# CatchMan1/AI-education-generative-recommendation

Hardware: AMD Instinct MI355X
Metric: RQ-VAE items encoded/s + SASRec seqs scored/s @1/8 GPU; HR@10/NDCG@10 parity (higher is better)
Workload: dtype f32; 1 GPU; rq_c2: RQ-VAE get_indices, 3x256 codebooks, in 768 -> [256,128] -> e 32, data-derived codebooks, BERT-statistics item embeddings; global_batch=100000, parallelism=item-sharded x1, no collective

## Files before the change

ai-education-generative-recommendation_amd/csrc/abi.cpp:

```cpp
#include <atomic>
#include <cstring>
#include <string>

#include "gr_common.h"

namespace gr {
static thread_local std::string g_last_error;
void set_error(const std::string& msg) { g_last_error = msg; }
void clear_error() { g_last_error.clear(); }

int cu_count() {
  static int cus = 0;
  if (!cus) {
    int dev = 0;
    if (hipGetDevice(&dev) != hipSuccess) dev = 0;
    if (hipDeviceGetAttribute(&cus, hipDeviceAttributeMultiprocessorCount, dev) != hipSuccess || cus < 1)
      cus = 256;
  }
  return cus;
}

struct Opt {
  const char* name;
  std::atomic<int64_t>* v;
  int64_t lo, hi;
};
static std::atomic<int64_t> g_rq_fused{1};
static std::atomic<int64_t> g_sas_fused{2};
static std::atomic<int64_t> g_sas_rowtile{1};
static std::atomic<int64_t> g_lin_wres{1};
static std::atomic<int64_t> g_emb_proj{1};
static std::atomic<int64_t> g_topk_half{2};
static std::atomic<int64_t> g_attn_k16{1};
static std::atomic<int64_t> g_rq_filter{1};
static std::atomic<int64_t> g_rq_tail_merge{1};

static std::atomic<int64_t> g_kmeans_small{1};
static std::atomic<int64_t> g_bert_tile{0};

static const Opt kOpts[] = {
    {"rq_fused", &g_rq_fused, 0, 1},   {"sas_fused", &g_sas_fused, 0, 3}, {"sas_rowtile", &g_sas_rowtile, 0, 1},
    {"lin_wres", &g_lin_wres, 0, 1},   {"emb_proj", &g_emb_proj, 0, 1},   {"topk_half", &g_topk_half, 0, 2},
    {"attn_k16", &g_attn_k16, 0, 1},   {"rq_filter", &g_rq_filter, 0, 1}, {"kmeans_small", &g_kmeans_small, 0, 1},
    {"rq_tail_merge", &g_rq_tail_merge, 0, 1}, {"bert_tile", &g_bert_tile, 0, 3},
};

static const Opt* find_opt(const char* name) {
  for (const Opt& o : kOpts)
    if (!strcmp(name, o.name)) return &o;
  return nullptr;
}

int64_t option(const char* name) {
  const Opt* o = find_opt(name);
  return o ? o->v->load() : -1;
}
}

extern "C" int gr_set_option(const char* name, int64_t value) {
  gr::clear_error();
  if (!name) return gr::fail(GR_ERR_ARG, "gr_set_option: null name");
  const gr::Opt* o = gr::find_opt(name);
  if (!o || value < o->lo || value > o->hi)
    return gr::fail(GR_ERR_ARG, std::string("gr_set_option: unknown option or value: ") + name);
  o->v->store(value);
  return GR_OK;
}

extern "C" int64_t gr_get_option(const char* name) { return name ? gr::option(name) : -1; }

extern "C" const char* gr_version(void) { return "gr_amd 0.1.0 gfx950"; }
extern "C" const char* gr_last_error(void) { return gr::g_last_error.c_str(); }
```

ai-education-generative-recommendation_amd/csrc/rq.hip:

```cpp
#include <atomic>

#include "gr_common.h"
#include "rq_fused.h"
#include "rq_quant.h"

#ifndef GR_QDIAG
#define GR_QDIAG 0
#endif

#ifndef GR_QRES
#define GR_QRES 1
#endif

namespace gr {

struct RQLevels {
  const float* cb[GR_MAX_LEVELS];
  int K[GR_MAX_LEVELS];
};

constexpr int RQ_SPLIT_MAX = 3;
constexpr size_t RQ_PART_BYTES = 2 * RQ_SPLIT_MAX * 4 * 32 * 3 * sizeof(float);

template <int EP>
// ... 118 lines not shown
    }
    __syncthreads();
  }
  int loff = 0;
  for (int l = 0; l < (GR_QDIAG == 5 ? 0 : L); ++l) {
    const int K = lv.K[l];
    const float* cb = lv.cb[l];
    float* cbi = resident ? cbs + loff * EP : cbs;
    float* cni = resident ? cns + loff : cns;
    const int kst = resident ? K : kch;
    loff += (K + 31) & ~31;
    float rn[RQ_MAXT], best[RQ_MAXT], second[RQ_MAXT];
    int bi[RQ_MAXT];
#pragma unroll
    for (int i = 0; i < RQ_MAXT; ++i) {
      rn[i] = GR_QDIAG == 4 ? 0.f : rn_exact<EP>(res[i], e, h);
      best[i] = __builtin_inff();
      second[i] = __builtin_inff();
      bi[i] = 0x7fffffff;
    }
    const int c_last = ((K - 1) / kst) * kst;
    for (int c0 = 0; c0 < K; c0 += kst) {
      const int cnt = min(kst, K - c0);
      if (!resident) {
        __syncthreads();
        stage_codes<EP, NT, FULL>(cb, e, c0, cnt, cbs, cns, tid);
      }
      const int ct_n = (cnt + 31) >> 5;
      const int q_lo = simd * ct_n / 4, q_hi = (simd + 1) * ct_n / 4;
#pragma unroll 1
      for (int ct = 0; ct < ct_n; ++ct) {
        const bool in_q = ct >= q_lo && ct < q_hi;
        const int code = min(ct * 32 + r, cnt - 1);
        f32x4 a[HQ];
#pragma unroll
        for (int j = 0; j < HQ; ++j)
          a[j] = *reinterpret_cast<const f32x4*>(cbi + cb_off<EP>(code, HQ * h + j));
        float cnv[16];
#pragma unroll
        for (int g4 = 0; g4 < 4; ++g4) {
          const f32x4 q = *reinterpret_cast<const f32x4*>(cni + ct * 32 + 8 * g4 + 4 * h);
#pragma unroll
          for (int i = 0; i < 4; ++i) cnv[4 * g4 + i] = q[i];
        }
#pragma unroll
        for (int i = 0; i < RQ_MAXT; ++i) {
          if (i < my && (!is_split(i) || in_q)) {
            f32x16 acc;
#pragma unroll
            for (int v = 0; v < 16; ++v) acc[v] = 0.f;
#pragma unroll
            for (int j = 0; j < HQ; ++j)
#pragma unroll
              for (int s = 0; s < 4; ++s) {
                if (GR_QDIAG == 2) acc[4 * j + s] += a[j][s] * res[i][j][s];
                else acc = mfma32(a[j][s], res[i][j][s], acc);
              }
#pragma unroll
            for (int v = 0; v < 16; ++v) {
              const int cd = c0 + ct * 32 + (v & 3) + 8 * (v >> 2) + 4 * h;
              const float dd = fmaf(-2.f, acc[v], rn[i] + cnv[v]);
              if (GR_QDIAG == 1) {
                best[i] = fminf(best[i], acc[v]);
                continue;
              }
              const bool lt = dd < best[i];
              if (SECOND) second[i] = lt ? best[i] : fminf(second[i], dd);
              bi[i] = lt ? cd : bi[i];
              best[i] = lt ? dd : best[i];
            }
          }
        }
      }
    }
#pragma unroll
    for (int i = 0; i < RQ_MAXT; ++i) {
      if (i < my) {
        const float ob = __shfl_xor(best[i], 32), os = __shfl_xor(second[i], 32);
        const int oi = __shfl_xor(bi[i], 32);
        merge_min<SECOND>(best[i], second[i], bi[i], ob, os, oi);
      }
    }
    if (split_plan) {
      float* pl = part + (l & 1) * (RQ_SPLIT_MAX * 4 * 32 * 3);
#pragma unroll
      for (int i = 0; i < RQ_MAXT; ++i)
        if (i < my && is_split(i) && h == 0) {
          float* ep = pl + (((wk + i * WS - base) * 4 + simd) * 32 + r) * 3;
          ep[0] = best[i];
          ep[1] = second[i];
          ep[2] = __int_as_float(bi[i]);
        }
      __syncthreads();
#pragma unroll
      for (int i = 0; i < RQ_MAXT; ++i)
        if (i < my && is_split(i)) {
          const float* ep = pl + ((wk + i * WS - base) * 4 * 32 + r) * 3;
          float bb = ep[0], ss = ep[1];
          int ii = __float_as_int(ep[2]);
#pragma unroll
          for (int q = 1; q < 4; ++q)
            merge_min<SECOND>(bb, ss, ii, ep[q * 96], ep[q * 96 + 1], __float_as_int(ep[q * 96 + 2]));
          best[i] = bb;
          second[i] = ss;
          bi[i] = ii;
        }
    }
#pragma unroll
    for (int i = 0; i < RQ_MAXT; ++i) {
      if (i < my) {
        int b = bi[i];
        if (b >= K) b = 0;
        const int64_t item = (int64_t)tile_of(i) * 32 + r;
        if (h == 0 && item < n && (!is_split(i) || simd == 0)) {
          idx_out[item * L + l] = (int64_t)b;
          if (best_out) best_out[item * L + l] = best[i];
          if (gap_out) gap_out[item * L + l] = second[i] - best[i];
        }
        f32x4 cw[HQ];
        if (b >= c_last) {
#pragma unroll
          for (int j = 0; j < HQ; ++j)
            cw[j] = *reinterpret_cast<const f32x4*>(cbi + cb_off<EP>(b - c_last, HQ * h + j));
        } else {
#pragma unroll
          for (int j = 0; j < HQ; ++j)
#pragma unroll
            for (int s = 0; s < 4; ++s) {
              const int f = 8 * j + 2 * s + h;
              cw[j][s] = f < e ? cb[(int64_t)b * e + f] : 0.f;
            }
        }
#pragma unroll
        for (int j = 0; j < HQ; ++j)
#pragma unroll
          for (int s = 0; s < 4; ++s) {
            const float xq = res[i][j][s] + (cw[j][s] - res[i][j][s]);
            res[i][j][s] = res[i][j][s] - xq;
          }
      }
    }
  }
}

#ifndef GR_FDIAG
#define GR_FDIAG 0
#endif
#ifndef GR_FSB
#define GR_FSB 1
#endif
#ifndef GR_FLIVE
#define GR_FLIVE 1
#endif

typedef __bf16 bf16x8 __attribute__((ext_vector_type(8)));

constexpr int RQF_KMAX = 1024;
constexpr int RQF_F32_KMAX = 512;

__device__ __forceinline__ void split_bf16(float x, __bf16& hi, __bf16& lo) {
#pragma clang fp contract(off)
  hi = (__bf16)x;
  lo = (__bf16)(x - (float)hi);
}

__device__ __forceinline__ f32x16 filter_tile(const bf16x8 (&ah)[2], const bf16x8 (&al)[2], const bf16x8 (&bh)[2],
                                              const bf16x8 (&bl)[2], f32x16 acc) {
#pragma unroll
  for (int t = 0; t < 2; ++t) acc = __builtin_amdgcn_mfma_f32_32x32x16_bf16(ah[t], bh[t], acc, 0, 0, 0);
#pragma unroll
  for (int t = 0; t < 2; ++t) acc = __builtin_amdgcn_mfma_f32_32x32x16_bf16(ah[t], bl[t], acc, 0, 0, 0);
#pragma unroll
  for (int t = 0; t < 2; ++t) acc = __builtin_amdgcn_mfma_f32_32x32x16_bf16(al[t], bh[t], acc, 0, 0, 0);
  return acc;
}

__host__ __device__ inline size_t filter_lds_floats(int kch, int f32_lds) {
  return ((size_t)kch * 32 * (f32_lds ? 2 : 1) + (size_t)kch + 16 + 255) & ~(size_t)255;
}
#ifndef GR_FDMA
#define GR_FDMA 1
#endif
__device__ __forceinline__ void filter_stage_dma(const float* __restrict__ img, float* buf, int img_floats, int tid) {
  const int w = __builtin_amdgcn_readfirstlane(tid >> 6), lane = tid & 63;
  for (int c = w; c < img_floats / 256; c += RQ_W)
    __builtin_amdgcn_global_load_lds(
        reinterpret_cast<const __attribute__((address_space(1))) void*>(reinterpret_cast<uintptr_t>(img + c * 256 + lane * 4)),
        (__attribute__((address_space(3))) void*)(buf + c * 256), 16, 0, 0);
}
template <bool LIVE>
__device__ __forceinline__ void filter_stage(const float* __restrict__ cb, int K, int kch, int f32_lds, float* sm,
                                             const float* __restrict__ img, int img_floats, int tid) {
#pragma clang fp contract(off)
  constexpr int EP = 32, W = RQ_W, NT = W * 64;
  if (img) {
    for (int f = tid; f < img_floats / 4; f += NT)
      *reinterpret_cast<f32x4*>(sm + 4 * f) = *reinterpret_cast<const f32x4*>(img + 4 * f);
    return;
  }
  float* bimg = sm;
  float* cns = bimg + kch * EP;
  float* wmax = cns + kch;
  float* fimg = wmax + 16;
  const int lane = tid & 63, w = tid >> 6, ct_n = (K + 31) >> 5;
  for (int f = tid; f < 2 * K; f += NT) {
    const int c = f >> 1, t = f & 1;
    float x[16];
#pragma unroll
    for (int q = 0; q < 4; ++q) {
      const f32x4 v = *reinterpret_cast<const f32x4*>(cb + (int64_t)c * EP + 16 * t + 4 * q);
#pragma unroll
      for (int i = 0; i < 4; ++i) x[4 * q + i] = v[i];
    }
#pragma unroll
    for (int hh = 0; hh < 2; ++hh) {
      bf16x8 vh, vl;
#pragma unroll
      for (int i = 0; i < 8; ++i) {
        __bf16 a, b;
        split_bf16(x[(i < 4 ? 2 * i : 8 + 2 * (i - 4)) + hh], a, b);
        vh[i] = a;
        vl[i] = b;
      }
      *reinterpret_cast<bf16x8*>(bimg + cb_off<EP>(c, 2 * hh + t)) = vh;
      *reinterpret_cast<bf16x8*>(bimg + cb_off<EP>(c, 4 + 2 * hh + t)) = vl;
    }
  }
  if (f32_lds) stage_rows<EP, NT, true>(cb, EP, 0, K, fimg, tid);
  float cmax = 0.f;
  for (int c = tid; c < (LIVE ? 256 : ct_n * 32); c += NT) {
    float s = __builtin_inff();
    if (c < K) {
      const float* row = cb + (int64_t)c * EP;
      s = aten_rowsq([&](int f) { return row[f]; }, EP);
      cmax = fmaxf(cmax, s);
    }
    cns[c] = s;
  }
  cmax = xmax<32>(xmax<16>(xmax<8>(xmax<4>(xmax<2>(xmax<1>(cmax))))));
  if (lane == 0) wmax[w] = cmax;
}

template <bool LIVE, bool TAIL, bool DBUF>
__global__ __launch_bounds__(RQ_W * 64) void rq_filter_kernel(
    const float* __restrict__ z, int64_t n, int L, RQLevels lv, int kch, int f32_lds,
    int64_t* __restrict__ idx_out, int tiles, uint32_t* __restrict__ cand_out, RqPending tail,
    const float* __restrict__ img, int img_floats) {
#pragma clang fp contract(off)
  constexpr int EP = 32, HQ = 4, W = RQ_W, MAXT = GR_FMAXT;
  if (LIVE) f32_lds = 1;
  extern __shared__ __attribute__((aligned(16))) float sm[];
  const int tid = threadIdx.x, lane = tid & 63, w = tid >> 6, r = lane & 31, h = lane >> 5;
  const int left = TAIL ? tail.left : 0;
  const bool owner = TAIL && (int)blockIdx.x < left;
  int t_begin, t_end;
  rq_filter_range(tiles, (int)gridDim.x, left, (int)blockIdx.x, t_begin, t_end);
  const int cm = t_end - t_begin, lt = TAIL ? tail.t0 + (int)blockIdx.x : 0;
  const int my = (cm + (owner ? 1 : 0) - w + W - 1) / W;
  auto tile_at = [&](int i) -> int { return (TAIL && w + i * W >= cm) ? lt : t_begin + w + i * W; };

  if constexpr (TAIL) {
    if (owner) {
      using FC = FusedCfg<256, 128>;
      float *h1s = sm, *h2s = h1s + FT * FC::P1, *w3s = h2s + FT * FC::P2;
      rq_leftover_tile<256, 128, true>(tail.h1g + (int64_t)blockIdx.x * FT * 256, n, lt, tail.W2, tail.b2, tail.W3,
                                       tail.b3, tail.z, h1s, h2s, w3s, h1s);
      __syncthreads();
    }
  }

  f32x4 res[MAXT][HQ];
#pragma unroll
  for (int i = 0; i < MAXT; ++i) {
    const int64_t item = (int64_t)tile_at(i) * 32 + r;
    const bool ok = i < my && item < n;
    const int64_t ic = ok ? item : 0;
    if (TAIL && owner && i < my && w + i * W == cm) {
#pragma unroll
      for (int j = 0; j < HQ; ++j) {
        const f32x4 lo = *reinterpret_cast<const f32x4*>(sm + r * ZLP + 8 * j);
        const f32x4 hi = *reinterpret_cast<const f32x4*>(sm + r * ZLP + 8 * j + 4);
        const f32x4 v = h ? f32x4{lo[1], lo[3], hi[1], hi[3]} : f32x4{lo[0], lo[2], hi[0], hi[2]};
        res[i][j] = ok ? v : f32x4{0.f, 0.f, 0.f, 0.f};
      }
      continue;
    }
#pragma unroll
    for (int j = 0; j < HQ; ++j) {
      const f32x4 lo = *reinterpret_cast<const f32x4*>(z + ic * EP + 8 * j);
      const f32x4 hi = *reinterpret_cast<const f32x4*>(z + ic * EP + 8 * j + 4);
      const f32x4 v = h ? f32x4{lo[1], lo[3], hi[1], hi[3]} : f32x4{lo[0], lo[2], hi[0], hi[2]};
      res[i][j] = ok ? v : f32x4{0.f, 0.f, 0.f, 0.f};
    }
  }

  for (int l = 0; l < L; ++l) {
    const int K = lv.K[l];
    const float* __restrict__ cb = lv.cb[l];
    const int ct_n = (K + 31) >> 5;
    if (DBUF) asm volatile("s_waitcnt vmcnt(0)" ::: "memory");
    __syncthreads();
    float* lb = sm;
    if constexpr (DBUF) {
      lb = sm + (l & 1) * img_floats;
      if (l == 0) {
        filter_stage_dma(img, lb, img_floats, tid);
        asm volatile("s_waitcnt vmcnt(0)" ::: "memory");
        __syncthreads();
      }
      if (l + 1 < L) filter_stage_dma(img + (size_t)(l + 1) * img_floats, sm + ((l + 1) & 1) * img_floats, img_floats, tid);
    } else {
      filter_stage<LIVE>(cb, K, kch, f32_lds, sm, img ? img + (size_t)l * img_floats : nullptr, img_floats, tid);
    }
    float* bimg = lb;
    float* cns = bimg + kch * EP;
    float* wmax = cns + kch;
    float* fimg = wmax + 16;
    float cmax = 0.f;
    if (!DBUF) __syncthreads();
#pragma unroll
    for (int i = 0; i < W; ++i) cmax = fmaxf(cmax, wmax[i]);

    float rn[MAXT], m[MAXT];
#pragma unroll
    for (int i = 0; i < MAXT; ++i) {
      if (!LIVE) rn[i] = rn_exact<EP>(res[i], EP, h);
      m[i] = __builtin_inff();
    }
    auto split_res = [&](int i, bf16x8 (&bh)[2], bf16x8 (&bl)[2]) {
#pragma unroll
      for (int t = 0; t < 2; ++t)
#pragma unroll
        for (int q = 0; q < 8; ++q) {
          __bf16 a, b;
          split_bf16(-2.f * res[i][2 * t + (q >> 2)][q & 3], a, b);
          bh[t][q] = a;
          bl[t][q] = b;
        }
    };
    auto load_codes = [&](int ct, bf16x8 (&ah)[2], bf16x8 (&al)[2], f32x16& cnv) {
      const int code = min(ct * 32 + r, K - 1);
#pragma unroll
      for (int t = 0; t < 2; ++t) {
        ah[t] = *reinterpret_cast<const bf16x8*>(bimg + cb_off<EP>(code, 2 * h + t));
        al[t] = *reinterpret_cast<const bf16x8*>(bimg + cb_off<EP>(code, 4 + 2 * h + t));
      }
#pragma unroll
      for (int g4 = 0; g4 < 4; ++g4) {
        const f32x4 q = *reinterpret_cast<const f32x4*>(cns + ct * 32 + 8 * g4 + 4 * h);
#pragma unroll
        for (int i = 0; i < 4; ++i) cnv[4 * g4 + i] = q[i];
      }
    };
    float thr[MAXT], best[MAXT];
    int bi[MAXT];
    bool allm[MAXT];
    uint32_t ncand[MAXT];
#pragma unroll
    for (int i = 0; i < MAXT; ++i) {
      best[i] = __builtin_inff();
      bi[i] = 0x7fffffff;
      ncand[i] = 0;
    }
    auto set_thr = [&](int i) {
      m[i] = fminf(m[i], __shfl_xor(m[i], 32));
      thr[i] = m[i] + 2.f * rq_filter_bound(rn[i], cmax);
      allm[i] = !(fabsf(thr[i]) < __builtin_inff());
      if (GR_FDIAG == 2) bi[i] = __float_as_int(thr[i]) & 0xff;
    };
    auto min16 = [](float t, const f32x16& a) {
#pragma unroll
      for (int v = 0; v < 16; v += 2) t = fminf(fminf(t, a[v]), a[v + 1]);
      return t;
    };
    auto mark16 = [](uint32_t k, const f32x16& a, float th) {
      const f32x16 d = th - a;
#pragma unroll
      for (int v = 0; v < 16; ++v) k = __builtin_amdgcn_alignbit(k, __float_as_uint(d[v]), 31);
      return k;
    };
    auto walk = [&](int i, int g0, const uint32_t (&nm)[4]) {
      if (GR_FDIAG == 1) {
        bi[i] = min(bi[i], (int)((nm[0] ^ nm[1] ^ nm[2] ^ nm[3]) >> 1));
        return;
      }
      uint32_t cm[4];
#pragma unroll
      for (int q = 0; q < 4; ++q) cm[q] = allm[i] ? 0xffffffffu : ~nm[q];
      if (__builtin_amdgcn_ballot_w64((cm[0] | cm[1] | cm[2] | cm[3]) != 0) == 0) return;
      float ev[16], od[16];
#pragma unroll
      for (int j = 0; j < HQ; ++j)
#pragma unroll
        for (int s = 0; s < 4; ++s) {
          const float own = res[i][j][s], oth = __shfl_xor(own, 32);
          ev[4 * j + s] = h ? oth : own;
          od[4 * j + s] = h ? own : oth;
        }
      while (__builtin_amdgcn_ballot_w64((cm[0] | cm[1] | cm[2] | cm[3]) != 0) != 0) {
        const int q = cm[0] ? 0 : cm[1] ? 1 : cm[2] ? 2 : 3;
        const uint32_t wd = cm[0] ? cm[0] : cm[1] ? cm[1] : cm[2] ? cm[2] : cm[3];
        const bool act = wd != 0;
        const int p = 31 - __clz((int)(wd | 1u));
        const uint32_t keep = ~(1u << p);
#pragma unroll
        for (int qq = 0; qq < 4; ++qq) cm[qq] = qq == q ? cm[qq] & keep : cm[qq];
        const int v = 15 - (p & 15);
        const int cd = (g0 + 2 * q + (p < 16 ? 1 : 0)) * 32 + (v & 3) + 8 * (v >> 2) + 4 * h;
        if (act && cd < K) {
          float cr[EP];
          if (f32_lds) {
#pragma unroll
            for (int sl = 0; sl < 2 * HQ; ++sl) {
              const f32x4 t = *reinterpret_cast<const f32x4*>(fimg + cb_off<EP>(cd, sl));
#pragma unroll
              for (int s = 0; s < 4; ++s) cr[8 * (sl % HQ) + 2 * s + sl / HQ] = t[s];
            }
          } else {
#pragma unroll
            for (int sl = 0; sl < EP / 4; ++sl) {
              const f32x4 t = *reinterpret_cast<const f32x4*>(cb + (int64_t)cd * EP + 4 * sl);
#pragma unroll
              for (int s = 0; s < 4; ++s) cr[4 * sl + s] = t[s];
            }
          }
          float chain = 0.f;
#pragma unroll
          for (int k = 0; k < EP; ++k) chain = fmaf(cr[k], (k & 1) ? od[k >> 1] : ev[k >> 1], chain);
          const float dd = fmaf(-2.f, chain, rn[i] + cns[cd]);
          const bool lt = dd < best[i];
          bi[i] = lt ? cd : bi[i];
          best[i] = lt ? dd : best[i];
          ++ncand[i];
        }
      }
    };
    auto finish = [&](int i) {
      float sec = 0.f;
      merge_min<false>(best[i], sec, bi[i], __shfl_xor(best[i], 32), 0.f, __shfl_xor(bi[i], 32));
      int b = bi[i];
      if (b >= K || b < 0) b = 0;
      const int64_t item = (int64_t)tile_at(i) * 32 + r;
      if (h == 0 && item < n) idx_out[item * L + l] = (int64_t)b;
      if (GR_FDIAG == 3) {
        const uint32_t tot = ncand[i] + __shfl_xor(ncand[i], 32);
        if (h == 0 && item < n && cand_out) cand_out[item * L + l] = tot;
      }
      f32x4 cw[HQ];
      if (f32_lds) {
#pragma unroll
        for (int j = 0; j < HQ; ++j) cw[j] = *reinterpret_cast<const f32x4*>(fimg + cb_off<EP>(b, HQ * h + j));
      } else {
#pragma unroll
        for (int j = 0; j < HQ; ++j) {
          const f32x4 lo = *reinterpret_cast<const f32x4*>(cb + (int64_t)b * EP + 8 * j);
          const f32x4 hi = *reinterpret_cast<const f32x4*>(cb + (int64_t)b * EP + 8 * j + 4);
          cw[j] = h ? f32x4{lo[1], lo[3], hi[1], hi[3]} : f32x4{lo[0], lo[2], hi[0], hi[2]};
        }
      }
#pragma unroll
      for (int j = 0; j < HQ; ++j)
#pragma unroll
        for (int s = 0; s < 4; ++s) {
          const float xq = res[i][j][s] + (cw[j][s] - res[i][j][s]);
          res[i][j][s] = res[i][j][s] - xq;
        }
    };
    if constexpr (LIVE) {
#pragma unroll
      for (int i = 0; i < MAXT; ++i) {
        if (i < my && GR_FDIAG == 4) {
          rn[i] = 0.f;
          finish(i);
        } else if (i < my) {
          f32x16 acc[8];
          float t = __builtin_inff();
          bf16x8 bh[2], bl[2];
          split_res(i, bh, bl);
          rn[i] = rn_exact<EP>(res[i], EP, h);
#pragma unroll
          for (int u = 0; u < 8; ++u)
          {
            bf16x8 ah[2], al[2];
            f32x16 cnv;
            load_codes(u, ah, al, cnv);
            acc[u] = filter_tile(ah, al, bh, bl, cnv);
#if GR_FSB
            t = min16(t, acc[u]);
            __builtin_amdgcn_sched_barrier(0);
#endif
          }
#if !GR_FSB
#pragma unroll
          for (int u = 0; u < 8; ++u) t = min16(t, acc[u]);
#endif
          m[i] = t;
          set_thr(i);
          if (GR_FDIAG == 2) {
            finish(i);
            continue;
          }
          uint32_t nm[4];
#pragma unroll
          for (int u = 0; u < 8; ++u) {
            nm[u >> 1] = mark16((u & 1) ? nm[u >> 1] : 0u, acc[u], thr[i]);
            __builtin_amdgcn_sched_barrier(0);
          }
          walk(i, 0, nm);
          finish(i);
        }
      }
    } else {
      bf16x8 bh[MAXT][2], bl[MAXT][2];
#pragma unroll
      for (int i = 0; i < MAXT; ++i) split_res(i, bh[i], bl[i]);
#pragma unroll 1
      for (int ct = 0; ct < (GR_FDIAG == 4 ? 0 : ct_n); ++ct) {
        bf16x8 ah[2], al[2];
        f32x16 cnv;
        load_codes(ct, ah, al, cnv);
#pragma unroll
        for (int i = 0; i < MAXT; ++i)
          if (i < my) m[i] = min16(m[i], filter_tile(ah, al, bh[i], bl[i], cnv));
      }
#pragma unroll
      for (int i = 0; i < MAXT; ++i) set_thr(i);
      for (int g0 = 0; g0 < (GR_FDIAG == 2 || GR_FDIAG == 4 ? 0 : ct_n); g0 += 8) {
        uint32_t nmk[MAXT][4];
#pragma unroll
        for (int u = 0; u < 8; ++u) {
          if (g0 + u < ct_n) {
            bf16x8 ah[2], al[2];
            f32x16 cnv;
            load_codes(g0 + u, ah, al, cnv);
#pragma unroll
            for (int i = 0; i < MAXT; ++i)
              if (i < my)
                nmk[i][u >> 1] = mark16((u & 1) ? nmk[i][u >> 1] : 0u, filter_tile(ah, al, bh[i], bl[i], cnv), thr[i]);
          } else {
#pragma unroll
            for (int i = 0; i < MAXT; ++i) nmk[i][u >> 1] = (((u & 1) ? nmk[i][u >> 1] : 0u) << 16) | 0xffffu;
          }
        }
#pragma unroll
        for (int i = 0; i < MAXT; ++i)
          if (i < my) walk(i, g0, nmk[i]);
      }
#pragma unroll
      for (int i = 0; i < MAXT; ++i)
        if (i < my) finish(i);
    }
  }
}

template <bool LIVE>
__global__ __launch_bounds__(RQ_W * 64) void rq_cb_pack_kernel(RQLevels lv, int kch, int f32_lds,
                                                              float* __restrict__ out, int img_floats) {
  constexpr int W = RQ_W, NT = W * 64;
  extern __shared__ __attribute__((aligned(16))) float sm[];
  const int tid = threadIdx.x, l = blockIdx.x;
  for (int f = tid; f < img_floats; f += NT) sm[f] = 0.f;
  __syncthreads();
  filter_stage<LIVE>(lv.cb[l], lv.K[l], kch, f32_lds, sm, nullptr, 0, tid);
  __syncthreads();
  float* wmax = sm + kch * 32 + kch;
  float cmax = 0.f;
#pragma unroll
  for (int i = 0; i < W; ++i) cmax = fmaxf(cmax, wmax[i]);
  __syncthreads();
  if (tid < 16) wmax[tid] = tid < W ? cmax : 0.f;
  __syncthreads();
  for (int f = tid; f < img_floats; f += NT) out[(size_t)l * img_floats + f] = sm[f];
}

__global__ __launch_bounds__(256) void rq_code_norms_kernel(const float* __restrict__ cb, int K,
                                                            int e, float* __restrict__ cn) {
  const int c = blockIdx.x * 256 + threadIdx.x;
  if (c >= K) return;
  const float* row = cb + (int64_t)c * e;
  cn[c] = aten_rowsq([&](int f) { return row[f]; }, e);
}

static int launch_norms(const float* cb, int K, int e, float* cn, hipStream_t st) {
  hipLaunchKernelGGL(rq_code_norms_kernel, dim3((K + 255) / 256), dim3(256), 0, st, cb, K, e, cn);
  return check_launch("gr_rq_codebook_norms_f32");
}

template <int EP>
static int launch_quantize_e(const float* z, int64_t n, int e, int L, const RQLevels& lv, int64_t* idx,
                             float* best, float* gap, hipStream_t st) {
  int kmax = 0;
  for (int l = 0; l < L; ++l) kmax = lv.K[l] > kmax ? lv.K[l] : kmax;
  const int kch_max = 1024 * 32 / EP;
  int kch = ((kmax < kch_max ? kmax : kch_max) + 31) & ~31;
  const int64_t tiles = (n + 31) / 32;
  int ktot = 0;
  for (int l = 0; l < L; ++l) ktot += (lv.K[l] + 31) & ~31;
  const bool res = GR_QRES && tiles <= (int64_t)cu_count() &&
                   (size_t)ktot * EP * 4 + (size_t)ktot * 4 + RQ_PART_BYTES <= 160 * 1024;
  if (res) kch = ktot;
  const size_t lds = (size_t)kch * EP * 4 + (size_t)kch * 4 + RQ_PART_BYTES;
  int64_t grid = (int64_t)cu_count();
  const int64_t min_grid = (tiles + RQ_W * RQMaxT<EP>::value - 1) / (RQ_W * RQMaxT<EP>::value);
  if (grid < min_grid) grid = min_grid;
  if (grid > tiles) grid = tiles;
  if (grid > 0x7fffffffLL || tiles > 0x7fffffffLL) return fail(GR_ERR_UNSUPPORTED, "rq quantize: n too large");
  const bool full = e == EP;
  auto k = (best || gap) ? (full ? rq_quantize_kernel<EP, true, true> : rq_quantize_kernel<EP, true, false>)
                         : (full ? rq_quantize_kernel<EP, false, true> : rq_quantize_kernel<EP, false, false>);
  if (lds > 64 * 1024 &&
      hipFuncSetAttribute(reinterpret_cast<const void*>(k), hipFuncAttributeMaxDynamicSharedMemorySize,
                          (int)lds) != hipSuccess)
    return fail(GR_ERR_HIP, "rq quantize: cannot raise the LDS limit");
  hipLaunchKernelGGL(k, dim3((unsigned)grid), dim3(RQ_W * 64), lds, st, z, n, e, L, lv, kch, idx,
                     best, gap, (int)tiles, 1, res ? 1 : 0);
  return check_launch("gr_rq_quantize_f32");
}

static std::atomic<int64_t> g_filter_launches{0};
static std::atomic<uint32_t*> g_filter_counts{nullptr};

static bool filter_ok(int e, int L, const RQLevels& lv, const float* best, const float* gap) {
  if (e != 32 || best || gap || option("rq_filter") != 1) return false;
  for (int l = 0; l < L; ++l)
    if (lv.K[l] > RQF_KMAX) return false;
  return true;
}

static int64_t filter_grid(int64_t tiles, int64_t grid_in, int left) {
  const int cap = RQ_W * GR_FMAXT;
  int64_t grid = grid_in;
  const int64_t min_grid = (tiles + cap - 1) / cap;
  if (grid < min_grid) grid = min_grid;
  if (grid < left || left > tiles || tiles > 0x7fffffffLL) return 0;
  while (grid <= 0x7fffffffLL && rq_filter_max_count((int)tiles, (int)grid, left) > cap) ++grid;
  return grid > 0x7fffffffLL ? 0 : grid;
}

struct FilterShape {
  bool live;
  int kch, f32_lds;
  size_t floats;
};
static FilterShape filter_shape(int L, const RQLevels& lv) {
  int kmax = 0;
  for (int l = 0; l < L; ++l) kmax = lv.K[l] > kmax ? lv.K[l] : kmax;
  FilterShape s;
  s.live = GR_FLIVE && kmax <= 256;
  s.kch = s.live ? 256 : (kmax + 31) & ~31;
  s.f32_lds = s.kch <= RQF_F32_KMAX;
  s.floats = filter_lds_floats(s.kch, s.f32_lds);
  return s;
}

static int launch_filter(const float* z, int64_t n, int L, const RQLevels& lv, int64_t* idx, hipStream_t st,
                         const RqPending* tail = nullptr, const float* img = nullptr) {
  const FilterShape fs = filter_shape(L, lv);
  const bool live = fs.live;
  const int kch = fs.kch, f32_lds = fs.f32_lds;
  size_t lds = fs.floats * sizeof(float);
  const bool merged = tail && tail->h1g;
  const bool dbuf = GR_FDMA && live && img && L > 1 && 2 * lds <= 160 * 1024;
  if (dbuf) lds *= 2;
  if (merged && lds < FusedCfg<256, 128>::TAIL_LDS * sizeof(float)) lds = FusedCfg<256, 128>::TAIL_LDS * sizeof(float);
  const int64_t tiles = (n + 31) / 32;
  int64_t grid = (int64_t)cu_count();
  if (grid > tiles) grid = tiles;
  grid = filter_grid(tiles, grid, merged ? tail->left : 0);
  if (grid == 0)
    return fail(GR_ERR_UNSUPPORTED, merged ? "rq encode: n too large (the pending leftover tiles were not finished)"
                                           : "rq quantize: n too large");
  auto k = merged ? (live ? rq_filter_kernel<true, true, false> : rq_filter_kernel<false, true, false>)
                  : (live ? rq_filter_kernel<true, false, false> : rq_filter_kernel<false, false, false>);
#if GR_FDMA
  if (dbuf) k = merged ? rq_filter_kernel<true, true, true> : rq_filter_kernel<true, false, true>;
#endif
  if (lds > 64 * 1024 &&
      hipFuncSetAttribute(reinterpret_cast<const void*>(k),
                          hipFuncAttributeMaxDynamicSharedMemorySize, (int)lds) != hipSuccess)
    return fail(GR_ERR_HIP, merged ? "rq encode: cannot raise the LDS limit (the pending leftover tiles were not finished)"
                                   : "rq quantize: cannot raise the LDS limit");
  hipLaunchKernelGGL(k, dim3((unsigned)grid), dim3(RQ_W * 64), lds, st, z, n, L, lv, kch, f32_lds,
                     idx, (int)tiles, g_filter_counts.load(), merged ? *tail : RqPending{}, img, (int)fs.floats);
  g_filter_launches.fetch_add(1);
  return check_launch("gr_rq_quantize_f32");
}

static int launch_cb_pack(int L, const RQLevels& lv, float* out, hipStream_t st) {
  const FilterShape fs = filter_shape(L, lv);
  auto k = fs.live ? rq_cb_pack_kernel<true> : rq_cb_pack_kernel<false>;
  const size_t lds = fs.floats * sizeof(float);
  if (lds > 64 * 1024 &&
      hipFuncSetAttribute(reinterpret_cast<const void*>(k), hipFuncAttributeMaxDynamicSharedMemorySize, (int)lds) != hipSuccess)
    return fail(GR_ERR_HIP, "rq codebook pack: cannot raise the LDS limit");
  hipLaunchKernelGGL(k, dim3((unsigned)L), dim3(RQ_W * 64), lds, st, lv, fs.kch, fs.f32_lds, out, (int)fs.floats);
  return check_launch("gr_rq_codebook_pack_f32");
}

static int launch_quantize(const float* z, int64_t n, int e, int L, const RQLevels& lv,
                           int64_t* idx, float* best, float* gap, hipStream_t st, const float* img = nullptr) {
  if (n == 0) return GR_OK;
  if (filter_ok(e, L, lv, best, gap)) return launch_filter(z, n, L, lv, idx, st, nullptr, img);
  if (e <= 16) return launch_quantize_e<16>(z, n, e, L, lv, idx, best, gap, st);
  if (e <= 32) return launch_quantize_e<32>(z, n, e, L, lv, idx, best, gap, st);
  if (e <= 64) return launch_quantize_e<64>(z, n, e, L, lv, idx, best, gap, st);
  return fail(GR_ERR_UNSUPPORTED, "gr_rq_quantize_f32: e_dim must be <= 64");
}

static int check_levels(int32_t e, int32_t L, const int32_t* K, const float* const* cbs) {
  if (e < 1 || e > 4096) return fail(GR_ERR_UNSUPPORTED, "rq: 1 <= e_dim <= 4096");
  if (L < 1 || L > GR_MAX_LEVELS) return fail(GR_ERR_UNSUPPORTED, "rq: 1 <= L <= 8 levels");
  if (!K || !cbs) return fail(GR_ERR_ARG, "rq: null K / codebooks");
  for (int l = 0; l < L; ++l) {
    if (K[l] < 1) return fail(GR_ERR_ARG, "rq: codebook size must be >= 1");
    if (!cbs[l] || ((e == 16 || e == 32 || e == 64) && !aligned16(cbs[l]))) return fail(GR_ERR_ARG, "rq: codebooks must be 16-byte aligned");
  }
  return GR_OK;
}

static bool quant_chain(int64_t M, int e, int L, const int32_t* K) {
  if (e > 64) return false;
  for (int l = 0; l < L; ++l) {
    const MklPlan p = mkl_plan(M, e, K[l]);
    if (p.kind != MKL_CHAIN || p.kb < e) return false;
  }
  return true;
}

static bool mlp_chain(int64_t M, int32_t n_linear, const int32_t* dims) {
  for (int i = 0; i < n_linear; ++i) {
    const MklPlan p = mkl_plan(M, dims[i], dims[i + 1]);
    if (p.kind != MKL_CHAIN || p.kb % 2 != 0 || dims[i] % 4 != 0) return false;
  }
  return true;
}

}

extern "C" int32_t gr_mkl_plan(int64_t M, int32_t K, int32_t N, int32_t* kind, int32_t* kb) {
  const gr::MklPlan p = gr::mkl_plan(M, K, N);
  if (kind) *kind = p.kind;
  if (kb) *kb = p.kb;
  return gr::mkl_plan_pinned(M, K, N) ? 1 : 0;
}

extern "C" float gr_rq_filter_bound_f32(float rn, float cmax2) { return gr::rq_filter_bound(rn, cmax2); }

extern "C" int64_t gr_rq_filter_launches(void) { return gr::g_filter_launches.load(); }

extern "C" int gr_rq_filter_plan(int64_t tiles, int32_t grid_in, int32_t left, int32_t* begins_out,
                                 int32_t* counts_out, int32_t* grid_out) {
  using namespace gr;
  clear_error();
  if (tiles < 1 || grid_in < 1 || left < 0 || !grid_out) return fail(GR_ERR_ARG, "gr_rq_filter_plan: bad arguments");
  const int64_t grid = filter_grid(tiles, grid_in, left);
  if (grid == 0) return fail(GR_ERR_UNSUPPORTED, "gr_rq_filter_plan: left > grid or tiles, or too many tiles");
  *grid_out = (int32_t)grid;
  for (int b = 0; b < (int)grid && (begins_out || counts_out); ++b) {
    int mb, me;
    rq_filter_range((int)tiles, (int)grid, left, b, mb, me);
    if (begins_out) begins_out[b] = mb;
    if (counts_out) counts_out[b] = me - mb + (b < left ? 1 : 0);
  }
  return GR_OK;
}

extern "C" void gr_rq_filter_diag_counts(uint32_t* counts) { gr::g_filter_counts.store(counts); }

extern "C" int gr_rq_codebook_norms_f32(const float* codebook, int32_t K, int32_t e, float* cn_out,
                                        void* stream) {
  gr::clear_error();
  if (!codebook || !cn_out || K < 1 || e < 1) return gr::fail(GR_ERR_ARG, "gr_rq_codebook_norms_f32: bad args");
  return gr::launch_norms(codebook, K, e, cn_out, reinterpret_cast<hipStream_t>(stream));
}

extern "C" int gr_rq_quantize_f32(const float* z, int64_t n, int32_t e, int32_t L, const int32_t* K,
                                  const float* const* codebooks, const float* const* code_norms,
                                  int64_t* idx_out, float* best_out, float* gap_out,
                                  void* stream) {
  using namespace gr;
  clear_error();
  (void)code_norms;
  int rc = check_levels(e, L, K, codebooks);
  if (rc) return rc;
  if (n < 0) return fail(GR_ERR_ARG, "gr_rq_quantize_f32: n < 0");
  if (n == 0) return GR_OK;
  if (!z || !idx_out || ((e == 16 || e == 32 || e == 64) && !aligned16(z))) return fail(GR_ERR_ARG, "gr_rq_quantize_f32: bad pointer");
  if (!quant_chain(n, e, L, K)) {
    const int32_t dims[1] = {e};
    return gr_rq_rows_launch(z, n, n, nullptr, 0, 0, dims, nullptr, nullptr, nullptr, nullptr, nullptr, nullptr,
                             0.f, GR_ACT_NONE, L, K, codebooks, nullptr, idx_out, best_out, gap_out,
                             reinterpret_cast<hipStream_t>(stream));
  }
  RQLevels lv{};
  for (int l = 0; l < L; ++l) {
    lv.cb[l] = codebooks[l];
    lv.K[l] = K[l];
  }
  return launch_quantize(z, n, e, L, lv, idx_out, best_out, gap_out, reinterpret_cast<hipStream_t>(stream));
}

static size_t act_bytes(int64_t n, int32_t n_linear, const int32_t* dims) {
  int widest = 0;
  for (int i = 1; i <= n_linear; ++i) widest = dims[i] > widest ? dims[i] : widest;
  return gr::align_up((size_t)n * widest * 4, 256);
}

static size_t mlp_ws_bytes(int64_t n, int32_t n_linear, const int32_t* dims) {
  return 2 * act_bytes(n, n_linear, dims) + gr::align_up(gr_rq_fused_pack_floats(n_linear, dims) * 4, 256) + 256;
}

static int mlp_exact(const float* x, int64_t n, int32_t n_linear, const int32_t* dims, const float* const* weights,
                     const float* const* biases, const float* const* bn_mean, const float* const* bn_var,
                     const float* const* bn_w, const float* const* bn_b, float bn_eps, int32_t act, float* z_out,
                     void* workspace, hipStream_t st, const float* packed = nullptr,
                     gr::RqPending* pending = nullptr) {
  using namespace gr;
  if (!mlp_chain(n, n_linear, dims))
    return gr_rq_rows_launch(x, n, n, nullptr, 0, n_linear, dims, weights, biases, bn_mean, bn_var, bn_w, bn_b,
                             bn_eps, act, 0, nullptr, nullptr, z_out, nullptr, nullptr, nullptr, st);
  char* ws = reinterpret_cast<char*>(align_up(reinterpret_cast<uintptr_t>(workspace), 256));
  const size_t ab = act_bytes(n, n_linear, dims);
  float* buf[2] = {reinterpret_cast<float*>(ws), reinterpret_cast<float*>(ws + ab)};
  if (!bn_mean && act == GR_ACT_RELU && option("rq_fused") == 1) {
    const int rc = gr_rq_encoder_fused_launch(x, n, n_linear, dims, weights, biases, z_out,
                                              packed ? const_cast<float*>(packed) : reinterpret_cast<float*>(ws + 2 * ab),
                                              st, packed != nullptr, buf[0], pending);
    if (rc != GR_ERR_UNSUPPORTED) return rc;
    clear_error();
  }
  const float* cur = x;
  for (int i = 0; i < n_linear; ++i) {
    const bool last = i == n_linear - 1;
    float* out = last ? z_out : buf[i & 1];
    const bool bn = bn_mean && !last;
    const int rc = gr_linear_exact_launch(cur, n, dims[i], weights[i], dims[i + 1], biases ? biases[i] : nullptr,
// ... 189 lines not shown
```

ai-education-generative-recommendation_amd/csrc/rq_quant.h:

```cpp
#pragma once
#include "gr_common.h"

namespace gr {

template <int EP>
__device__ __forceinline__ int cb_off(int c, int q) {
  constexpr int S = EP / 4;
  constexpr int M = S >= 8 ? 7 : S - 1;
  return c * EP + 4 * (q ^ (c & M));
}

template <int EP>
__device__ __forceinline__ int feat_off(int c, int f) {
  return cb_off<EP>(c, (f & 1) * (EP / 8) + (f >> 3)) + ((f >> 1) & 3);
}

template <int EP>
__device__ __forceinline__ float rn_exact(const f32x4 (&rr)[EP / 8], int e, int h) {
#pragma clang fp contract(off)
  constexpr int HQ = EP / 8;
  const int nv = e >> 3, full = (nv >> 2) << 2, tail = e & 7;
  float A[4], T[4];
#pragma unroll
  for (int s = 0; s < 4; ++s) {
    float a0 = 0.f, a1 = 0.f, a2 = 0.f, a3 = 0.f;
    T[s] = 0.f;
#pragma unroll
    for (int v = 0; v < HQ; ++v) {
      const float x = rr[v][s];
      const float q = x * x;
      if (v < nv) {
        const int a = v < full ? (v & 3) : 0;
        if (a == 0) a0 = a0 + q;
        else if (a == 1) a1 = a1 + q;
        else if (a == 2) a2 = a2 + q;
        else a3 = a3 + q;
      } else if (v == nv) {
        T[s] = q;
      }
    }
    A[s] = ((a0 + a1) + a2) + a3;
  }
  float PA[4], PT[4];
#pragma unroll
  for (int s = 0; s < 4; ++s) {
    PA[s] = __shfl_xor(A[s], 32);
    PT[s] = __shfl_xor(T[s], 32);
  }
  if (e < 8) {
    float a0 = 0.f, a1 = 0.f, a2 = 0.f, a3 = 0.f;
#pragma unroll
    for (int i = 0; i < 7; ++i)
      if (i < e) {
        const float q = ((i & 1) == h) ? T[i >> 1] : PT[i >> 1];
        const int k = i < ((e >> 2) << 2) ? (i & 3) : 0;
        if (k == 0) a0 = a0 + q;
        else if (k == 1) a1 = a1 + q;
        else if (k == 2) a2 = a2 + q;
        else a3 = a3 + q;
      }
    return ((a0 + a1) + a2) + a3;
  }
  float f = 0.f;
#pragma unroll
  for (int jj = 0; jj < 7; ++jj)
    if (jj < tail) f = f + (((jj & 1) == h) ? T[jj >> 1] : PT[jj >> 1]);
#pragma unroll
  for (int jj = 0; jj < 8; ++jj) f = f + (((jj & 1) == h) ? A[jj >> 1] : PA[jj >> 1]);
  return f;
}

template <bool SECOND>
__device__ __forceinline__ void merge_min(float& best, float& second, int& bi, float ob, float os, int oi) {
  const bool take = (ob < best) | ((ob == best) & (oi < bi));
  if (SECOND) second = take ? fminf(os, best) : fminf(second, ob);
  best = take ? ob : best;
  bi = take ? oi : bi;
}

__host__ __device__ inline float rq_filter_bound(float rn, float cmax2) {
#pragma clang fp contract(off)
  const float R = __builtin_sqrtf(rn), C = __builtin_sqrtf(cmax2);
  return (0x1p-13f * (R * C) + 0x1p-15f * (rn + cmax2)) + 0x1p-116f * ((R + C) + 1.f);
}

}
```

Baseline: 271.8 million items/s.

## Skip exact rescoring when the bf16 filter leaves a single candidate code

In the RQ filter kernel, each row now counts the codes that survive the bf16 filter bound. When exactly one candidate survives, and the norms are small enough for the bound to be trustworthy, the row takes that code directly and skips the exact f32 distance walk. In the non-LIVE path, the lone candidate is held across code tiles and is re-evaluated only if more candidates appear later. This adds ballots and register state per tile, and an option rq_walk_all (default off) restores the old full walk.

```diff
diff --git a/ai-education-generative-recommendation_amd/csrc/abi.cpp b/ai-education-generative-recommendation_amd/csrc/abi.cpp
--- a/ai-education-generative-recommendation_amd/csrc/abi.cpp
+++ b/ai-education-generative-recommendation_amd/csrc/abi.cpp
@@ -34,6 +34,7 @@
 static std::atomic<int64_t> g_attn_k16{1};
 static std::atomic<int64_t> g_rq_filter{1};
 static std::atomic<int64_t> g_rq_tail_merge{1};
+static std::atomic<int64_t> g_rq_walk_all{0};
 
 static std::atomic<int64_t> g_kmeans_small{1};
 static std::atomic<int64_t> g_bert_tile{0};
@@ -43,6 +44,7 @@
     {"lin_wres", &g_lin_wres, 0, 1},   {"emb_proj", &g_emb_proj, 0, 1},   {"topk_half", &g_topk_half, 0, 2},
     {"attn_k16", &g_attn_k16, 0, 1},   {"rq_filter", &g_rq_filter, 0, 1}, {"kmeans_small", &g_kmeans_small, 0, 1},
     {"rq_tail_merge", &g_rq_tail_merge, 0, 1}, {"bert_tile", &g_bert_tile, 0, 3},
+    {"rq_walk_all", &g_rq_walk_all, 0, 1},
 };
 
 static const Opt* find_opt(const char* name) {
diff --git a/ai-education-generative-recommendation_amd/csrc/rq.hip b/ai-education-generative-recommendation_amd/csrc/rq.hip
--- a/ai-education-generative-recommendation_amd/csrc/rq.hip
+++ b/ai-education-generative-recommendation_amd/csrc/rq.hip
@@ -294,6 +294,9 @@
 #ifndef GR_FLIVE
 #define GR_FLIVE 1
 #endif
+#ifndef GR_FLAST
+#define GR_FLAST 0
+#endif
 
 typedef __bf16 bf16x8 __attribute__((ext_vector_type(8)));
 
@@ -387,7 +390,7 @@
 __global__ __launch_bounds__(RQ_W * 64) void rq_filter_kernel(
     const float* __restrict__ z, int64_t n, int L, RQLevels lv, int kch, int f32_lds,
     int64_t* __restrict__ idx_out, int tiles, uint32_t* __restrict__ cand_out, RqPending tail,
-    const float* __restrict__ img, int img_floats) {
+    const float* __restrict__ img, int img_floats, int walk_all) {
 #pragma clang fp contract(off)
   constexpr int EP = 32, HQ = 4, W = RQ_W, MAXT = GR_FMAXT;
   if (LIVE) f32_lds = 1;
@@ -498,6 +501,8 @@
     int bi[MAXT];
     bool allm[MAXT];
     uint32_t ncand[MAXT];
+    constexpr int HELD_NONE = -1, HELD_OPEN = -2;
+    int held[MAXT];
 #pragma unroll
     for (int i = 0; i < MAXT; ++i) {
       best[i] = __builtin_inff();
@@ -508,6 +513,7 @@
       m[i] = fminf(m[i], __shfl_xor(m[i], 32));
       thr[i] = m[i] + 2.f * rq_filter_bound(rn[i], cmax);
       allm[i] = !(fabsf(thr[i]) < __builtin_inff());
+      if (!LIVE) held[i] = (walk_all || allm[i] || !rq_lone_ok(rn[i], cmax)) ? HELD_OPEN : HELD_NONE;
       if (GR_FDIAG == 2) bi[i] = __float_as_int(thr[i]) & 0xff;
     };
     auto min16 = [](float t, const f32x16& a) {
@@ -521,6 +527,14 @@
       for (int v = 0; v < 16; ++v) k = __builtin_amdgcn_alignbit(k, __float_as_uint(d[v]), 31);
       return k;
     };
+    auto lowest = [&](const uint32_t (&cm)[4], int g0, int& q, uint32_t& keep) -> int {
+      q = cm[0] ? 0 : cm[1] ? 1 : cm[2] ? 2 : 3;
+      const uint32_t wd = cm[0] ? cm[0] : cm[1] ? cm[1] : cm[2] ? cm[2] : cm[3];
+      const int p = 31 - __clz((int)(wd | 1u));
+      keep = ~(1u << p);
+      const int v = 15 - (p & 15);
+      return (g0 + 2 * q + (p < 16 ? 1 : 0)) * 32 + (v & 3) + 8 * (v >> 2) + 4 * h;
+    };
     auto walk = [&](int i, int g0, const uint32_t (&nm)[4]) {
       if (GR_FDIAG == 1) {
         bi[i] = min(bi[i], (int)((nm[0] ^ nm[1] ^ nm[2] ^ nm[3]) >> 1));
@@ -529,7 +543,46 @@
       uint32_t cm[4];
 #pragma unroll
       for (int q = 0; q < 4; ++q) cm[q] = allm[i] ? 0xffffffffu : ~nm[q];
-      if (__builtin_amdgcn_ballot_w64((cm[0] | cm[1] | cm[2] | cm[3]) != 0) == 0) return;
+      int pend = -1;
+      if (!walk_all) {
+        int c = (__popc(cm[0]) + __popc(cm[1])) + (__popc(cm[2]) + __popc(cm[3]));
+        if (LIVE) c = (!allm[i] && rq_lone_ok(rn[i], cmax)) ? c : 2;
+        const uint64_t b1 = __builtin_amdgcn_ballot_w64(c >= 1), b2 = __builtin_amdgcn_ballot_w64(c >= 2);
+        const uint32_t any = (uint32_t)b1 | (uint32_t)(b1 >> 32);
+        const uint32_t two = (uint32_t)b2 | (uint32_t)(b2 >> 32) | ((uint32_t)b1 & (uint32_t)(b1 >> 32));
+        int q;
+        uint32_t keep;
+        const int cd = lowest(cm, g0, q, keep);
+        const int mine = (c == 1 && cd < K) ? cd : -1;
+        if constexpr (LIVE) {
+          if (!((two >> r) & 1)) {
+            bi[i] = mine >= 0 ? mine : bi[i];
+#pragma unroll
+            for (int qq = 0; qq < 4; ++qq) cm[qq] = 0u;
+          }
+        } else {
+          const uint64_t bh = __builtin_amdgcn_ballot_w64(held[i] >= 0);
+          const uint32_t hd = (uint32_t)bh | (uint32_t)(bh >> 32);
+          if (held[i] != HELD_OPEN) {
+            if (!((hd >> r) & 1)) {
+              if ((two >> r) & 1) {
+                held[i] = HELD_OPEN;
+              } else if ((any >> r) & 1) {
+                held[i] = mine >= 0 ? mine : HELD_NONE;
+#pragma unroll
+                for (int qq = 0; qq < 4; ++qq) cm[qq] = 0u;
+              }
+            } else if ((any >> r) & 1) {
+              pend = held[i];
+              held[i] = HELD_OPEN;
+            }
+          }
+        }
+      }
+      auto any_left = [&]() {
+        return __builtin_amdgcn_ballot_w64(((cm[0] | cm[1] | cm[2] | cm[3]) != 0) | (pend >= 0)) != 0;
+      };
+      if (!any_left()) return;
       float ev[16], od[16];
 #pragma unroll
       for (int j = 0; j < HQ; ++j)
@@ -539,16 +592,20 @@
           ev[4 * j + s] = h ? oth : own;
           od[4 * j + s] = h ? own : oth;
         }
-      while (__builtin_amdgcn_ballot_w64((cm[0] | cm[1] | cm[2] | cm[3]) != 0) != 0) {
-        const int q = cm[0] ? 0 : cm[1] ? 1 : cm[2] ? 2 : 3;
-        const uint32_t wd = cm[0] ? cm[0] : cm[1] ? cm[1] : cm[2] ? cm[2] : cm[3];
-        const bool act = wd != 0;
-        const int p = 31 - __clz((int)(wd | 1u));
-        const uint32_t keep = ~(1u << p);
+      while (any_left()) {
+        int q;
+        uint32_t keep;
+        int cd = lowest(cm, g0, q, keep);
+        bool act = (cm[0] | cm[1] | cm[2] | cm[3]) != 0;
+        if constexpr (!LIVE) {
+          const bool first = pend >= 0;
+          cd = first ? pend : cd;
+          keep = first ? 0xffffffffu : keep;
+          act = act || first;
+          pend = -1;
+        }
 #pragma unroll
         for (int qq = 0; qq < 4; ++qq) cm[qq] = qq == q ? cm[qq] & keep : cm[qq];
-        const int v = 15 - (p & 15);
-        const int cd = (g0 + 2 * q + (p < 16 ? 1 : 0)) * 32 + (v & 3) + 8 * (v >> 2) + 4 * h;
         if (act && cd < K) {
           float cr[EP];
           if (f32_lds) {
@@ -579,6 +636,9 @@
     };
     auto finish = [&](int i) {
       float sec = 0.f;
+      if constexpr (!LIVE) {
+        bi[i] = held[i] >= 0 ? held[i] : bi[i];
+      }
       merge_min<false>(best[i], sec, bi[i], __shfl_xor(best[i], 32), 0.f, __shfl_xor(bi[i], 32));
       int b = bi[i];
       if (b >= K || b < 0) b = 0;
@@ -588,6 +648,7 @@
         const uint32_t tot = ncand[i] + __shfl_xor(ncand[i], 32);
         if (h == 0 && item < n && cand_out) cand_out[item * L + l] = tot;
       }
+      if (GR_FLAST && l + 1 == L) return;
       f32x4 cw[HQ];
       if (f32_lds) {
 #pragma unroll
@@ -823,7 +884,8 @@
     return fail(GR_ERR_HIP, merged ? "rq encode: cannot raise the LDS limit (the pending leftover tiles were not finished)"
                                    : "rq quantize: cannot raise the LDS limit");
   hipLaunchKernelGGL(k, dim3((unsigned)grid), dim3(RQ_W * 64), lds, st, z, n, L, lv, kch, f32_lds,
-                     idx, (int)tiles, g_filter_counts.load(), merged ? *tail : RqPending{}, img, (int)fs.floats);
+                     idx, (int)tiles, g_filter_counts.load(), merged ? *tail : RqPending{}, img, (int)fs.floats,
+                     option("rq_walk_all") == 1 ? 1 : 0);
   g_filter_launches.fetch_add(1);
   return check_launch("gr_rq_quantize_f32");
 }
diff --git a/ai-education-generative-recommendation_amd/csrc/rq_quant.h b/ai-education-generative-recommendation_amd/csrc/rq_quant.h
--- a/ai-education-generative-recommendation_amd/csrc/rq_quant.h
+++ b/ai-education-generative-recommendation_amd/csrc/rq_quant.h
@@ -84,4 +84,9 @@
   return (0x1p-13f * (R * C) + 0x1p-15f * (rn + cmax2)) + 0x1p-116f * ((R + C) + 1.f);
 }
 
+__host__ __device__ inline bool rq_lone_ok(float rn, float cmax2) {
+#pragma clang fp contract(off)
+  return rn + cmax2 < 0x1p125f;
 }
+
+}
```

Result: no change. 271.8 million items/s (-0.0%).
